# bdaiinstitute/vlfm

Hardware: AMD Instinct MI355X
Metric: env-steps/s (VLM+value-map update), 640x480 RGB-D (higher is better)
Workload: dtype f16 ViT-g (f32 accumulate) + f32 Q-Former (split-f16, 22-bit); f32 confidence + f64 value maps; 1 GPU; configs[1] step x resident envs: BLIP-2 ITC + ValueMap+ObstacleMap+sort_waypoints; envs_per_gpu=256, global_envs=256, map=1000x1000 @ 20 px/m, parallelism=env-sharded x1, tuned_gemms=True, vit_gemm=hip:fc1, attention=hip

## Files before the change

### include/vlfm_amd.h

```cpp
#ifndef VLFM_AMD_H
#define VLFM_AMD_H

#include <stddef.h>
#include <stdint.h>

#ifdef __cplusplus
extern "C" {
#endif

typedef enum {
    VLFM_OK = 0,
    VLFM_ERR_INVALID = -1,
    VLFM_ERR_OUTSIDE_MAP = -2,
    VLFM_ERR_INDEX = -3,
    VLFM_ERR_HIP = -4,
    VLFM_ERR_CAPACITY = -5
} vlfm_status;

enum { VLFM_FUSE_DEFAULT = 0, VLFM_FUSE_REPLACE = 1, VLFM_FUSE_EQUAL_WEIGHTING = 2 };

const char* vlfm_last_error(void);
int vlfm_abi_version(void);

int vlfm_profile_enable(int on);
// ... 124 lines not shown
                                const int32_t* d_hbounds, const int32_t* d_hk, int hksize,
                                const int32_t* d_vbounds, const int32_t* d_vk, int vksize,
                                const float* h_mean3, const float* h_std3, uint8_t* d_tmp, void* d_out,
                                int out_dtype, int patch_size, void* stream);

int vlfm_itc_head_batched(const float* d_proj, int batch, int n_query, int proj_dim,
                          const float* d_text, float* d_out, void* stream);

#define VLFM_ITC_MAX_PROMPTS 8
int vlfm_itc_head_multi(const float* d_proj, int batch, int n_query, int proj_dim, const float* d_text_table, int n_text,
                        const int32_t* d_text_index, int n_prompts, float* d_out, void* stream);

int vlfm_layernorm_bias_f16(const void* d_x, const float* d_channel_bias, const void* d_gamma, const void* d_beta,
                            void* d_y, int rows, int dim, float eps, void* stream);

int vlfm_vit_attention_f16(const void* d_qkv, void* d_out, int batch, int tokens, int heads, int head_dim, float scale,
                           void* stream);

int vlfm_gemm_f16_nt(const void* d_x, const void* d_w, const void* d_bias, void* d_c, int m, int n, int k, int epilogue,
                     void* stream);

int vlfm_gemm_f16_pair_f32_nt(const void* d_x, const void* d_w_pair, const void* d_bias_f32, void* d_out, int m, int n_out, int k,
                              void* stream);

int vlfm_qformer_cross_attention_f32(const void* d_q, const void* d_kv_blocks, void* d_out, int batch, int tokens, int queries,
                                     int heads, int k_block0, int v_block0, int m_total, float scale, void* stream);

int vlfm_gemm_f16_tile_order(int m, int n, int group_m, int* out, int capacity_pairs);
int vlfm_gemm_f16_work_items(int m, int n, int grid, int* out, int capacity_pairs);

int vlfm_split_f32_to_f16_pair(const float* d_src, void* d_hi, void* d_lo, long long count, int* d_overflow, void* stream);
int vlfm_gemm_f32_nt(const float* d_x, const float* d_w, const float* d_bias, const float* d_residual, float* d_c, int m, int n,
                     int k, int activation, int precision, const void* d_w_hi, const void* d_w_lo, int* d_overflow, void* stream);


int vlfm_layernorm_rows_f32(const float* d_x, const float* d_gamma, const float* d_beta, float* d_out, int batch, int height,
                            int width, int channels, int window, float eps, void* stream);
int vlfm_window_reverse_add_f32(float* d_x, const float* d_windows, int batch, int height, int width, int channels, int window,
                                void* stream);
int vlfm_dwconv3x3_nhwc_f32(const float* d_x, const float* d_w9c, const float* d_bias, float* d_out, int batch, int height, int width,
                            int channels, void* stream);
int vlfm_window_attention_f32(const float* d_qkv, const float* d_bias_t, float* d_out, long long windows, int tokens, int heads,
                              float scale, void* stream);
int vlfm_layernorm_rows_shifted_f32(const float* d_x, const float* d_gamma, const float* d_beta, float* d_out, int batch, int height,
                                    int width, int channels, int window, float eps, int shift, int pad_zero, void* stream);
int vlfm_window_reverse_add_shifted_f32(float* d_x, const float* d_windows, int batch, int height, int width, int channels, int window,
                                        int shift, void* stream);
int vlfm_window_attention_masked_f32(const float* d_qkv, const float* d_bias_t, const float* d_mask_t, int windows_per_image, float* d_out,
                                     long long windows, int tokens, int heads, float scale, void* stream);

int vlfm_maxpool2x2_nhwc_f16(const void* d_x, void* d_out, int batch, int height, int width, int channels, void* stream);
int vlfm_conv_nhwc_tile(int pixels, int cin, int cout, int ksize, int* tile_pixels, int* tile_channels);
int vlfm_conv_nhwc_f16(const void* d_x, const void* d_w, const void* d_bias, void* d_out, const void* d_zero, int batch,
                       int height, int width, int cin, int cout, int ksize, int stride, int x_pix_stride,
                       int out_pix_stride, int act, void* stream);

int vlfm_resize_area_tab_host(int ssize, int dsize, int32_t* h_first, int32_t* h_count, float* h_w, int ktaps_capacity);

int vlfm_resize_area_batched(const uint8_t* d_rgb, int n, int height, int width, int out_h, int out_w,
                             const int32_t* d_xfirst, const int32_t* d_xcount, const float* d_xw, int xktaps,
                             const int32_t* d_yfirst, const int32_t* d_ycount, const float* d_yw, int yktaps,
                             void* d_out, int out_dtype, void* stream);

int vlfm_to_tensor_normalize_batched(const uint8_t* d_rgb, int n, int height, int width, const float* h_mean3,
                                     const float* h_std3, float* d_out, void* stream);

// ... 218 lines not shown
```

### vlfm_amd/_lib.py

```python
from __future__ import annotations

import ctypes
import os
import subprocess
from typing import Optional

_HERE = os.path.dirname(os.path.abspath(__file__))
LIB_PATH = os.path.join(_HERE, "libvlfm_amd.so")
SOURCES = ["value_map.hip", "depth_ingest.hip", "depth_holes.hip", "obstacle_map.hip", "vlm_ops.hip", "vit_attention.hip", "qformer_attention.hip", "detect_ops.hip", "object_cloud.hip", "cloud_query.hip", "gemm_f16.hip", "gemm_f32.hip", "conv_nhwc.hip", "sam_ops.hip", "map_render.hip", "jpeg_codec.hip", "jpeg_entropy.hip", "jpeg_decode.hip", "world_render.hip", "geodesic.hip", "map_planner.hip", "host.cpp"]

VLFM_OK = 0
VLFM_ERR_INVALID = -1
VLFM_ERR_OUTSIDE_MAP = -2
VLFM_ERR_INDEX = -3
VLFM_ERR_HIP = -4
VLFM_ERR_CAPACITY = -5

FUSION_TYPES = {"default": 0, "replace": 1, "equal_weighting": 2}


class VmPose(ctypes.Structure):
    _fields_ = [("inv_affine", ctypes.c_double * 6), ("row0", ctypes.c_int32), ("col0", ctypes.c_int32),
                ("env", ctypes.c_int32), ("reserved", ctypes.c_int32)]


class IngestParams(ctypes.Structure):
    _fields_ = [("tf", ctypes.c_double * 12), ("depth_scale", ctypes.c_float), ("depth_offset", ctypes.c_float),
                ("depth_max", ctypes.c_float), ("reserved0", ctypes.c_float), ("fx", ctypes.c_double),
                ("fy", ctypes.c_double), ("min_height", ctypes.c_double), ("max_height", ctypes.c_double),
                ("env", ctypes.c_int32), ("scatter", ctypes.c_int32)]


FOG_MAX_POLY = 80


class FogParams(ctypes.Structure):
    _fields_ = [("env", ctypes.c_int32), ("ax", ctypes.c_int32), ("ay", ctypes.c_int32), ("radius", ctypes.c_int32),
                ("n_poly", ctypes.c_int32), ("reserved", ctypes.c_int32), ("rot_c", ctypes.c_double),
                ("rot_s", ctypes.c_double), ("line_len", ctypes.c_double), ("poly", ctypes.c_longlong * (2 * FOG_MAX_POLY))]


class ScatterJournal(ctypes.Structure):
    _fields_ = [("d_cells", ctypes.c_void_p), ("d_count", ctypes.c_void_p), ("capacity", ctypes.c_int32),
# ... 48 lines not shown
        obj = os.path.join(objdir, os.path.basename(src) + ".o")
        if not os.path.exists(obj) or os.path.getmtime(obj) < max(os.path.getmtime(src), hdr_time):
            cmd = ["hipcc"] + flags + ["-c", src, "-o", obj]
            if verbose:
                print(" ".join(cmd), flush=True)
            subprocess.check_call(cmd)
        return obj

    with ThreadPoolExecutor(max_workers=min(8, len(srcs))) as pool:
        objs = list(pool.map(compile_one, srcs))
    if os.path.exists(LIB_PATH) and all(os.path.getmtime(LIB_PATH) >= os.path.getmtime(o) for o in objs):
        return LIB_PATH
    cmd = ["hipcc", "--offload-arch=gfx950", "-shared", "-fPIC", "-o", LIB_PATH] + objs
    if verbose:
        print(" ".join(cmd), flush=True)
    subprocess.check_call(cmd)
    return LIB_PATH


_lib: Optional[ctypes.CDLL] = None


def lib() -> ctypes.CDLL:
    global _lib
    if _lib is None:
        if not os.path.exists(LIB_PATH):
            raise ImportError(
                f"{LIB_PATH} is missing: build it with `python -c 'import __graft_entry__ as g; g.build()'` "
                "(hipcc --offload-arch=gfx950).  vlfm_amd has no CPU fallback.")
        L = ctypes.CDLL(LIB_PATH)
        vp, ci, cd = ctypes.c_void_p, ctypes.c_int, ctypes.c_double
        L.vlfm_last_error.restype = ctypes.c_char_p
        L.vlfm_abi_version.restype = ci
        L.vlfm_profile_enable.argtypes = [ci]
        L.vlfm_host_wait_mode.argtypes = [ci]
        L.vlfm_profile_read.argtypes = [ctypes.c_char_p, ctypes.POINTER(cd), ctypes.POINTER(ci)]
        L.vlfm_value_map_pose_params.argtypes = [vp, vp, vp, ci, ci, ci, ci, vp, ctypes.POINTER(ci)]
        L.vlfm_cone_template_host.argtypes = [cd, cd, ci, cd, vp, ci, vp, ci, ctypes.POINTER(ci)]
        L.vlfm_tan_table_host.argtypes = [cd, ci, vp]
        L.vlfm_disc_rows_host.argtypes = [ci, vp]
        L.vlfm_cone_template_build.argtypes = [vp, vp, ci, ci, vp, vp, vp]
        L.vlfm_depth_ingest_batched.argtypes = [vp, ci, ci, ci, vp, vp, vp, ci, ci, vp, vp, vp, vp, vp]
        L.vlfm_selftest_div_exact.argtypes = [vp, ci, cd, vp, vp]
        L.vlfm_hole_scratch_bytes.argtypes = [ci, ci, ci, ci, ci]
        L.vlfm_hole_scratch_bytes.restype = ctypes.c_size_t
        L.vlfm_fill_small_holes_batched.argtypes = [vp, vp, ci, ci, ci, cd, vp, ctypes.c_size_t, ci, ci, vp, vp, vp, vp,
                                                    ci, vp, vp]
        L.vlfm_depth_scatter_holes_batched.argtypes = [vp, ci, ci, ci, vp, vp, vp, vp, ci, ci, vp, vp, vp]
        L.vlfm_fill_small_holes_rig_batched.argtypes = [vp, vp, ci, ci, ci, cd, vp, ctypes.c_size_t, ci, ci, vp, vp, vp, vp,
                                                        ci, vp, vp, ci, vp]
        L.vlfm_depth_scatter_holes_rig_batched.argtypes = [vp, ci, ci, ci, vp, vp, vp, vp, ci, ci, vp, vp, vp, vp]
        L.vlfm_layernorm_bias_f16.argtypes = [vp, vp, vp, vp, vp, ci, ci, ctypes.c_float, vp]
        L.vlfm_vit_attention_f16.argtypes = [vp, vp, ci, ci, ci, ci, ctypes.c_float, vp]
        L.vlfm_gemm_f16_nt.argtypes = [vp, vp, vp, vp, ci, ci, ci, ci, vp]
        L.vlfm_gemm_f16_pair_f32_nt.argtypes = [vp, vp, vp, vp, ci, ci, ci, vp]
        L.vlfm_qformer_cross_attention_f32.argtypes = [vp, vp, vp, ci, ci, ci, ci, ci, ci, ci, ctypes.c_float, vp]
        L.vlfm_gemm_f32_nt.argtypes = [vp, vp, vp, vp, vp, ci, ci, ci, ci, ci, vp, vp, vp, vp]
        L.vlfm_split_f32_to_f16_pair.argtypes = [vp, vp, vp, ctypes.c_longlong, vp, vp]
        L.vlfm_layernorm_rows_f32.argtypes = [vp, vp, vp, vp, ci, ci, ci, ci, ci, ctypes.c_float, vp]
        L.vlfm_window_reverse_add_f32.argtypes = [vp, vp, ci, ci, ci, ci, ci, vp]
        L.vlfm_dwconv3x3_nhwc_f32.argtypes = [vp, vp, vp, vp, ci, ci, ci, ci, vp]
        L.vlfm_window_attention_f32.argtypes = [vp, vp, vp, ctypes.c_longlong, ci, ci, ctypes.c_float, vp]
        L.vlfm_layernorm_rows_shifted_f32.argtypes = [vp, vp, vp, vp, ci, ci, ci, ci, ci, ctypes.c_float, ci, ci, vp]
        L.vlfm_window_reverse_add_shifted_f32.argtypes = [vp, vp, ci, ci, ci, ci, ci, ci, vp]
        L.vlfm_window_attention_masked_f32.argtypes = [vp, vp, vp, ci, vp, ctypes.c_longlong, ci, ci, ctypes.c_float, vp]
        L.vlfm_maxpool2x2_nhwc_f16.argtypes = [vp, vp, ci, ci, ci, ci, vp]
        L.vlfm_conv_nhwc_tile.argtypes = [ci, ci, ci, ci, ctypes.POINTER(ci), ctypes.POINTER(ci)]
        L.vlfm_conv_nhwc_f16.argtypes = [vp, vp, vp, vp, vp, ci, ci, ci, ci, ci, ci, ci, ci, ci, ci, vp]
        L.vlfm_value_map_update_fused_batched.argtypes = [vp, ci, vp, vp, vp, ci, vp, vp, ci, vp, vp, ci, ci, ci, cd, cd,
                                                          ci, ci, vp, vp, vp, vp, vp]
        L.vlfm_value_map_update_rig_batched.argtypes = [vp, ci, vp, vp, vp, ci, ci, ci, vp, vp, vp, ci, ci, ci, ci, ci, vp, vp,
                                                        vp, vp]
        L.vlfm_value_map_sort_waypoints_batched.argtypes = [vp, ci, ci, vp, ci, ci, vp, ci, vp, vp]
        L.vlfm_resample_coeffs_host.argtypes = [ci, ci, vp, vp, ci, ctypes.POINTER(ci)]
        L.vlfm_resample_coeffs_filter_host.argtypes = [ci, ci, ci, vp, vp, ci, ctypes.POINTER(ci)]
        L.vlfm_preprocess_sam_batched.argtypes = [vp, ci, ci, ci, ci, ci, vp, vp, ci, vp, vp, ci, vp, vp, ci, vp, vp, vp]
        L.vlfm_preprocess_rgb_batched.argtypes = [vp, ci, ci, ci, ci, vp, vp, ci, vp, vp, ci, vp, vp, vp, vp, ci, ci, vp]
        L.vlfm_itc_head_batched.argtypes = [vp, ci, ci, ci, vp, vp, vp]
        L.vlfm_itc_head_multi.argtypes = [vp, ci, ci, ci, vp, ci, vp, ci, vp, vp]
        cf = ctypes.c_float
        L.vlfm_resize_area_tab_host.argtypes = [ci, ci, vp, vp, vp, ci]
        L.vlfm_resize_area_batched.argtypes = [vp, ci, ci, ci, ci, ci, vp, vp, vp, ci, vp, vp, vp, ci, vp, ci, vp]
        L.vlfm_to_tensor_normalize_batched.argtypes = [vp, ci, ci, ci, vp, vp, vp, vp]
        L.vlfm_nms_scratch_bytes.argtypes = [ci]
        L.vlfm_nms_scratch_bytes.restype = ctypes.c_size_t
        L.vlfm_nms.argtypes = [vp, vp, ci, cf, vp, ctypes.c_size_t, vp, vp, ci, vp]
        L.vlfm_ms_deform_attn.argtypes = [vp, vp, vp, vp, vp, ci, ci, ci, ci, ci, ci, ci, vp, vp]
        L.vlfm_ms_deform_attn_fused.argtypes = [vp, vp, vp, vp, vp, ci, ci, ci, ci, ci, ci, ci, ci, vp, vp]
        L.vlfm_object_cloud_batch_scratch_bytes.argtypes = [ci, ci, ci]
        L.vlfm_object_cloud_batch_scratch_bytes.restype = ctypes.c_size_t
# ... 110 lines not shown
```

### vlfm_amd/csrc/gemm_f32.hip

```cpp
#include <hip/hip_runtime.h>
#include <stdint.h>
#include <stdlib.h>

#include "../../include/vlfm_amd.h"
#include "gelu_f16.h"
#include "mfma.h"
#include "profile.h"
#include "status.h"

namespace vlfm {
namespace g32 {

constexpr int TB = 128;
constexpr int TK = 32;
constexpr int ROWB = TK * 4;
constexpr int OPER = TB * ROWB;
constexpr int BUF = 2 * OPER;
constexpr int EPI_ROW = 272;
constexpr int EPI_WAVE = 64 * EPI_ROW;
constexpr int LDS_EXACT = 4 * EPI_WAVE > 2 * BUF ? 4 * EPI_WAVE : 2 * BUF;

enum { ACT_NONE = 0, ACT_RELU = 1, ACT_GELU = 2 };

struct Args {
    const float* x;
    const float* w;
    const float* bias;
    const float* residual;
    float* c;
    int M, N, K;
    int tiles_m, tiles_n;
    int* overflow;
    const _Float16* w_hi;
    const _Float16* w_lo;
};

__device__ inline void tile_of_block(const Args& a, int& tm, int& tn) {
    const int bid = xcd_contiguous(blockIdx.x, a.tiles_m * a.tiles_n);
    tm = bid / a.tiles_n;
    tn = bid - tm * a.tiles_n;
}

__device__ inline void stage_tile(const Args& a, lds_ptr lds, int buf, int n0, int m0, int k0, int wave, int lane) {
    const int sub = lane >> 3, p = lane & 7;
#pragma unroll
    for (int j = 0; j < 4; j++) {
        const int chunk = wave * 4 + j;
        const int r = chunk * 8 + sub;
        const int s4 = swz128(r, p) >> 2;
        const int rn = min(n0 + r, a.N - 1), rm = min(m0 + r, a.M - 1);
        const float* gw = a.w + (size_t)rn * a.K + k0 + s4;
        const float* gx = a.x + (size_t)rm * a.K + k0 + s4;
        const int dst = __builtin_amdgcn_readfirstlane(buf + chunk * 1024);
        __builtin_amdgcn_global_load_lds((gbl_ptr)gw, lds + dst, 16, 0, 0);
        __builtin_amdgcn_global_load_lds((gbl_ptr)gx, lds + dst + OPER, 16, 0, 0);
    }
}

template <bool SPLIT>
__device__ inline void store_tile(const Args& a, unsigned char* smem, const floatx16 (&acc)[2][2], const floatx16 (&cross)[2][2],
                                  int act, int wave, int wn, int wm, int lane, int m0, int n0) {
    unsigned char* stg = smem + wave * EPI_WAVE;
    const int c32 = lane & 31, h4 = (lane >> 5) * 4;
    floatx4 bias4[2][4];
#pragma unroll
    for (int i = 0; i < 2; i++)
#pragma unroll
        for (int g = 0; g < 4; g++) {
            floatx4 b = {0.f, 0.f, 0.f, 0.f};
            if (a.bias) {
                const int n = n0 + wn * 64 + i * 32 + g * 8 + h4;
                if (n + 4 <= a.N && ((uintptr_t)a.bias & 15) == 0) b = *reinterpret_cast<const floatx4*>(a.bias + n);
                else
                    for (int e = 0; e < 4; e++) b[e] = n + e < a.N ? a.bias[n + e] : 0.f;
            }
            bias4[i][g] = b;
        }
#pragma unroll
    for (int i = 0; i < 2; i++)
#pragma unroll
        for (int g = 0; g < 4; g++) {
            const int nl = i * 32 + g * 8 + h4;
            const floatx4 b = bias4[i][g];
#pragma unroll
            for (int j = 0; j < 2; j++) {
                floatx4 v;
#pragma unroll
                for (int e = 0; e < 4; e++) {
                    float t = acc[i][j][g * 4 + e];
                    if (SPLIT) t = fmaf(cross[i][j][g * 4 + e], 0x1p-11f, t);
                    t += b[e];
                    if (act == ACT_RELU) t = fmaxf(t, 0.f);
                    else if (act == ACT_GELU) t = gelu_erf(t);
                    v[e] = t;
                }
                *reinterpret_cast<floatx4*>(stg + (j * 32 + c32) * EPI_ROW + nl * 4) = v;
            }
        }
    wait_lgkmcnt0();
    const int rsub = lane >> 4, chunk = lane & 15;
    const bool vec = (a.N & 3) == 0;
    const int n = n0 + wn * 64 + chunk * 4;
    const bool fast = vec && n + 4 <= a.N;
    floatx4 r[16], v[16];
#pragma unroll
    for (int it = 0; it < 16; it++) {
        const int m = m0 + wm * 64 + it * 4 + rsub;
        r[it] = floatx4{0.f, 0.f, 0.f, 0.f};
        if (a.residual && fast && m < a.M) r[it] = *reinterpret_cast<const floatx4*>(a.residual + (size_t)m * a.N + n);
    }
#pragma unroll
    for (int it = 0; it < 16; it++) v[it] = *reinterpret_cast<const floatx4*>(stg + (it * 4 + rsub) * EPI_ROW + chunk * 16);
#pragma unroll
    for (int it = 0; it < 16; it++) {
        const int m = m0 + wm * 64 + it * 4 + rsub;
        if (m >= a.M || n >= a.N) continue;
        const size_t at = (size_t)m * a.N + n;
        if (fast) {
            *reinterpret_cast<floatx4*>(a.c + at) = v[it] + r[it];
        } else {
            for (int e = 0; e < 4 && n + e < a.N; e++) a.c[at + e] = v[it][e] + (a.residual ? a.residual[at + e] : 0.f);
        }
    }
}

__global__ __launch_bounds__(256, 2) void gemm_f32_exact_kernel(Args a, int act) {
    extern __shared__ __attribute__((aligned(16))) unsigned char smem[];
    lds_ptr lds = (lds_ptr)smem;
    const int tid = threadIdx.x, lane = tid & 63;
    const int wave = __builtin_amdgcn_readfirstlane(tid >> 6);
    const int wn = wave >> 1, wm = wave & 1;
    int tm, tn;
    tile_of_block(a, tm, tn);
    const int m0 = tm * TB, n0 = tn * TB;
    const int NT = a.K / TK;

    floatx16 acc[2][2];
#pragma unroll
    for (int i = 0; i < 2; i++)
#pragma unroll
        for (int j = 0; j < 2; j++)
#pragma unroll
            for (int e = 0; e < 16; e++) acc[i][j][e] = 0.f;

    stage_tile(a, lds, 0, n0, m0, 0, wave, lane);
    wait_vmcnt<0>();
    __builtin_amdgcn_s_barrier();
    asm volatile("" ::: "memory");
// ... 3 lines not shown
        const int cur = (t & 1) * BUF;
        if (t + 1 < NT) stage_tile(a, lds, cur ^ BUF, n0, m0, (t + 1) * TK, wave, lane);
#pragma unroll
        for (int kk = 0; kk < 4; kk++) {
            const int s = kk * 2 + h;
            floatx4 fa[2], fb[2];
#pragma unroll
            for (int i = 0; i < 2; i++) {
                const int R = wn * 64 + i * 32 + r32;
                fa[i] = *reinterpret_cast<const floatx4*>(smem + cur + R * ROWB + swz128(R, s));
            }
#pragma unroll
            for (int j = 0; j < 2; j++) {
                const int R = wm * 64 + j * 32 + r32;
                fb[j] = *reinterpret_cast<const floatx4*>(smem + cur + OPER + R * ROWB + swz128(R, s));
            }
#pragma unroll
            for (int q = 0; q < 4; q++)
#pragma unroll
                for (int i = 0; i < 2; i++)
#pragma unroll
                    for (int j = 0; j < 2; j++)
                        acc[i][j] = __builtin_amdgcn_mfma_f32_32x32x2f32(fa[i][q], fb[j][q], acc[i][j], 0, 0, 0);
        }
        wait_vmcnt<0>();
        __builtin_amdgcn_s_barrier();
        asm volatile("" ::: "memory");
    }
    store_tile<false>(a, smem, acc, acc, act, wave, wn, wm, lane, m0, n0);
}

constexpr int SROWB = TK * 2;
constexpr int SOPER = TB * SROWB;
constexpr int SBUF = 4 * SOPER;

__device__ inline int sslot(int row, int slot) { return (slot ^ ((row >> 2) & 3)) << 4; }

__device__ inline void split4(const floatx4 v, half4& hi, half4& lo, bool& over) {
#pragma unroll
    for (int e = 0; e < 4; e++) {
        const float a = v[e];
        over |= !(fabsf(a) < 65504.0f);
        const _Float16 hh = (_Float16)a;
        hi[e] = hh;
        lo[e] = (_Float16)((a - (float)hh) * 2048.0f);
    }
}

constexpr int XO = 0, WO = 2 * SOPER;
constexpr int LDS_SPLIT = 4 * EPI_WAVE > 2 * SBUF ? 4 * EPI_WAVE : 2 * SBUF;

__global__ __launch_bounds__(256, 2) void gemm_f32_split_kernel(Args a, int act) {
    extern __shared__ __attribute__((aligned(16))) unsigned char smem[];
    lds_ptr lds = (lds_ptr)smem;
    const int tid = threadIdx.x, lane = tid & 63;
    const int wave = __builtin_amdgcn_readfirstlane(tid >> 6);
    const int wn = wave >> 1, wm = wave & 1;
    int tm, tn;
    tile_of_block(a, tm, tn);
    const int m0 = tm * TB, n0 = tn * TB;
    const int NT = a.K / TK;

    floatx16 acc[2][2], crs[2][2];
#pragma unroll
    for (int i = 0; i < 2; i++)
#pragma unroll
        for (int j = 0; j < 2; j++)
#pragma unroll
            for (int e = 0; e < 16; e++) { acc[i][j][e] = 0.f; crs[i][j][e] = 0.f; }

    floatx4 xr[4];
    bool over = false;
    auto load_x = [&](int k0) {
#pragma unroll
        for (int u = 0; u < 4; u++) {
            const int idx = tid + 256 * u, r = idx >> 3, pc = idx & 7;
            const int rm = min(m0 + r, a.M - 1);
            xr[u] = *reinterpret_cast<const floatx4*>(a.x + (size_t)rm * a.K + k0 + pc * 4);
        }
    };
    auto put_x = [&](int buf) {
#pragma unroll
        for (int u = 0; u < 4; u++) {
            const int idx = tid + 256 * u, r = idx >> 3, pc = idx & 7;
            half4 hi, lo;
            split4(xr[u], hi, lo, over);
            const int off = r * SROWB + sslot(r, pc >> 1) + (pc & 1) * 8;
            *reinterpret_cast<half4*>(smem + buf + XO + off) = hi;
            *reinterpret_cast<half4*>(smem + buf + XO + SOPER + off) = lo;
        }
    };
    auto stage_w = [&](int buf, int k0) {
        const int sub = lane >> 2, p = lane & 3;
#pragma unroll
        for (int j = 0; j < 2; j++) {
            const int chunk = wave * 2 + j;
            const int r = chunk * 16 + sub;
            const int s = p ^ ((r >> 2) & 3);
            const int rn = min(n0 + r, a.N - 1);
            const size_t g = (size_t)rn * a.K + k0 + s * 8;
            const int dst = __builtin_amdgcn_readfirstlane(buf + WO + chunk * 1024);
            __builtin_amdgcn_global_load_lds((gbl_ptr)(a.w_hi + g), lds + dst, 16, 0, 0);
            __builtin_amdgcn_global_load_lds((gbl_ptr)(a.w_lo + g), lds + dst + SOPER, 16, 0, 0);
        }
    };

    load_x(0);
    stage_w(0, 0);
    put_x(0);
    wait_vmcnt<0>();
    wait_lgkmcnt0();
    __builtin_amdgcn_s_barrier();
    asm volatile("" ::: "memory");

    const int r32 = lane & 31, h = lane >> 5;
    for (int t = 0; t < NT; t++) {
        const int cur = (t & 1) * SBUF;
        if (t + 1 < NT) {
            load_x((t + 1) * TK);
            stage_w(cur ^ SBUF, (t + 1) * TK);
        }
#pragma unroll
        for (int kk = 0; kk < 2; kk++) {
            const int s = kk * 2 + h;
            half8 whi[2], wlo[2], xhi[2], xlo[2];
#pragma unroll
            for (int i = 0; i < 2; i++) {
                const int R = wn * 64 + i * 32 + r32, o = cur + WO + R * SROWB + sslot(R, s);
                whi[i] = *reinterpret_cast<const half8*>(smem + o);
                wlo[i] = *reinterpret_cast<const half8*>(smem + o + SOPER);
            }
#pragma unroll
            for (int j = 0; j < 2; j++) {
                const int R = wm * 64 + j * 32 + r32, o = cur + XO + R * SROWB + sslot(R, s);
                xhi[j] = *reinterpret_cast<const half8*>(smem + o);
                xlo[j] = *reinterpret_cast<const half8*>(smem + o + SOPER);
            }
#pragma unroll
            for (int i = 0; i < 2; i++)
#pragma unroll
                for (int j = 0; j < 2; j++) {
                    acc[i][j] = __builtin_amdgcn_mfma_f32_32x32x16_f16(whi[i], xhi[j], acc[i][j], 0, 0, 0);
                    crs[i][j] = __builtin_amdgcn_mfma_f32_32x32x16_f16(whi[i], xlo[j], crs[i][j], 0, 0, 0);
                    crs[i][j] = __builtin_amdgcn_mfma_f32_32x32x16_f16(wlo[i], xhi[j], crs[i][j], 0, 0, 0);
                }
        }
        if (t + 1 < NT) put_x(cur ^ SBUF);
        wait_vmcnt<0>();
        wait_lgkmcnt0();
        __builtin_amdgcn_s_barrier();
        asm volatile("" ::: "memory");
    }
    if (over && a.overflow) atomicOr(a.overflow, 1);
    store_tile<true>(a, smem, acc, crs, act, wave, wn, wm, lane, m0, n0);
}

__global__ void split_f32_kernel(const float* __restrict__ src, _Float16* __restrict__ hi, _Float16* __restrict__ lo, long long n,
                                 int* overflow) {
    const long long i = (long long)blockIdx.x * blockDim.x + threadIdx.x;
    if (i >= n) return;
    const float a = src[i];
    if (!(fabsf(a) < 65504.0f) && overflow) atomicOr(overflow, 1);
    const _Float16 hh = (_Float16)a;
    hi[i] = hh;
    lo[i] = (_Float16)((a - (float)hh) * 2048.0f);
}

}
}

using namespace vlfm;
using namespace vlfm::g32;

extern "C" int vlfm_split_f32_to_f16_pair(const float* d_src, void* d_hi, void* d_lo, long long count, int* d_overflow, void* stream) {
    if (count == 0) return VLFM_OK;
    if (!d_src || !d_hi || !d_lo || count < 0) return fail(VLFM_ERR_INVALID, "split_f32_to_f16_pair: bad argument");
    const long long blocks = (count + 255) / 256;
    VLFM_KLAUNCH(split_f32_kernel, dim3((unsigned)blocks), dim3(256), 0, (hipStream_t)stream, d_src, (_Float16*)d_hi, (_Float16*)d_lo,
                 count, d_overflow);
    return check_launch("split_f32_kernel");
}

extern "C" int vlfm_gemm_f32_nt(const float* d_x, const float* d_w, const float* d_bias, const float* d_residual, float* d_c, int m,
                                int n, int k, int activation, int precision, const void* d_w_hi, const void* d_w_lo,
                                int* d_overflow, void* stream) {
    if (m == 0 || n == 0) return VLFM_OK;
    if (!d_x || !d_w || !d_c || m < 0 || n < 0 || k <= 0 || (k % TK) != 0 || activation < 0 || activation > 2 || precision < 0 ||
        precision > 1)
        return fail(VLFM_ERR_INVALID, "gemm_f32_nt: K must be a multiple of 32, activation 0..2, precision 0..1");
    if (((uintptr_t)d_x | (uintptr_t)d_w | (uintptr_t)d_c | (uintptr_t)d_residual | (uintptr_t)d_w_hi | (uintptr_t)d_w_lo) & 15)
        return fail(VLFM_ERR_INVALID, "gemm_f32_nt: X, W, C, residual and the split weights must be 16-byte aligned");
    if (precision == 1 && (!d_w_hi || !d_w_lo || !d_overflow))
        return fail(VLFM_ERR_INVALID, "gemm_f32_nt: the split form needs the pre-split weights and the overflow flag");
    Args a;
    a.x = d_x; a.w = d_w; a.bias = d_bias; a.residual = d_residual; a.c = d_c;
    a.M = m; a.N = n; a.K = k;
    a.tiles_m = (m + TB - 1) / TB; a.tiles_n = (n + TB - 1) / TB;
    a.overflow = d_overflow; a.w_hi = (const _Float16*)d_w_hi; a.w_lo = (const _Float16*)d_w_lo;
    if ((long long)a.tiles_m * a.tiles_n > 0x7fffffffLL) return fail(VLFM_ERR_CAPACITY, "gemm_f32_nt: too many tiles");
    const dim3 grid(a.tiles_m * a.tiles_n), block(256);
    static LdsOptIn opt_exact, opt_split;
    if (precision == 0) {
        if (LDS_EXACT > 64 * 1024 && !opt_exact.ensure(reinterpret_cast<const void*>(gemm_f32_exact_kernel), LDS_EXACT))
            return fail(VLFM_ERR_HIP, "gemm_f32_nt: cannot opt in to the LDS size");
        VLFM_TIMED("gemm_f32_exact_kernel", stream);
        VLFM_KLAUNCH(gemm_f32_exact_kernel, grid, block, LDS_EXACT, (hipStream_t)stream, a, activation);
        return check_launch("gemm_f32_exact_kernel");
    }
    if (LDS_SPLIT > 64 * 1024 && !opt_split.ensure(reinterpret_cast<const void*>(gemm_f32_split_kernel), LDS_SPLIT))
        return fail(VLFM_ERR_HIP, "gemm_f32_nt: cannot opt in to the LDS size");
    VLFM_TIMED("gemm_f32_split_kernel", stream);
    VLFM_KLAUNCH(gemm_f32_split_kernel, grid, block, LDS_SPLIT, (hipStream_t)stream, a, activation);
    return check_launch("gemm_f32_split_kernel");
}
```

### vlfm_amd/csrc/host.cpp

```cpp
#include <cmath>
#include <cstdint>
#include <cstring>
#include <mutex>
#include <string>

#include "../../include/vlfm_amd.h"
#include "status.h"

namespace vlfm {
static thread_local std::string g_last_error;
void set_last_error(const char* msg) { g_last_error = msg ? msg : ""; }
}

extern "C" const char* vlfm_last_error(void) { return vlfm::g_last_error.c_str(); }
extern "C" int vlfm_abi_version(void) { return 22; }

namespace {

const double kPi = 3.141592653589793238462643383279502884;

inline long round_half_even(double v) { return std::lrint(v); }

float sin_deg_table(int deg) {
    static float tab[451];
    static std::once_flag once;
    std::call_once(once, [] {
        for (int i = 0; i <= 450; i++) tab[i] = (float)(std::round(std::sin(i * kPi / 180.0) * 1e7) / 1e7);
    });
    return tab[deg];
}

}

extern "C" int vlfm_value_map_pose_params(const double* h_tf, const double* h_yaw, const int32_t* h_env, int n,
                                          int map_size, int pixels_per_meter, int template_size,
                                          vlfm_vm_pose* h_out, int* bad_index) {
    if (!h_tf || !h_out || n < 0 || map_size <= 0 || template_size <= 0)
        return vlfm::fail(VLFM_ERR_INVALID, "value_map_pose_params: bad argument");
    const double ppm = (double)pixels_per_meter;
    const int half = template_size / 2;
    for (int k = 0; k < n; k++) {
        const double* tf = h_tf + 16 * k;
        const double yaw = h_yaw ? h_yaw[k] : std::atan2(tf[4], tf[0]);
        const double degrees = (-yaw) * (180.0 / kPi);
        const double ang = degrees * (kPi / 180);
        const double alpha = std::cos(ang), beta = std::sin(ang);
        const double cx = (double)(float)half, cy = (double)(float)half;
        double M[6] = {alpha, beta, (1 - alpha) * cx - beta * cy, -beta, alpha, beta * cx + (1 - alpha) * cy};
// ... 245 lines not shown
```

### vlfm_amd/vlm/ops.py

```python
from __future__ import annotations

import ctypes
from typing import Dict, Optional, Tuple

import numpy as np
import torch

from .. import _lib

CLIP_MEAN = (0.48145466, 0.4578275, 0.40821073)
CLIP_STD = (0.26862954, 0.26130258, 0.27577711)
_DTYPE_CODE = {torch.float32: 0, torch.float16: 1, torch.bfloat16: 2}
_coeff_cache: Dict[Tuple[str, int, int], Tuple[torch.Tensor, torch.Tensor, int]] = {}


def _stream() -> int:
    return torch._C._cuda_getCurrentRawStream(torch._C._cuda_getDevice())


def resample_coeffs(in_size: int, out_size: int, bilinear: bool = False) -> Tuple[np.ndarray, np.ndarray, int]:
    bounds = np.zeros((out_size, 2), np.int32)
    cap = out_size * (2 * int(np.ceil(2.0 * max(1.0, in_size / out_size))) + 1)
    kk = np.zeros(cap, np.int32)
    ks = ctypes.c_int(0)
# ... 341 lines not shown
    if len(_split_cache) > 2048:
        for k in [k for k, v in _split_cache.items() if v[0]() is None]:
            del _split_cache[k]
    w = weight.detach().contiguous()
    hi = torch.empty(w.shape, dtype=torch.float16, device=w.device)
    lo = torch.empty_like(hi)
    bad = torch.zeros(1, dtype=torch.int32, device=w.device)
    _lib.check(_lib.lib().vlfm_split_f32_to_f16_pair(w.data_ptr(), hi.data_ptr(), lo.data_ptr(), w.numel(), bad.data_ptr(),
                                                     _stream()), "split_f32")
    gemm_f32_overflow_flag(w.device, owner).bitwise_or_(bad)
    _split_cache[key] = [weakref.ref(weight), tensor_version(weight), weight.data_ptr(), hi, lo, bad, False, owner]
    return hi, lo


def split_weights_bad(device, owner: str = "") -> bool:
    d = torch.device(device)
    entries = [v for v in _split_cache.values() if v[7] == owner and v[0]() is not None and v[5].device.type == d.type
               and (d.index is None or v[5].device.index == d.index)]
    if not entries:
        return False
    verdict = torch.cat([v[5] for v in entries]).cpu().tolist()
    for v, b in zip(entries, verdict):
        v[6] = bool(b)
    return any(verdict)


def linear_f32_supported(x: torch.Tensor, weight: torch.Tensor) -> bool:
    k = weight.shape[1]
    return (x.is_cuda and x.dtype == torch.float32 and weight.dtype == torch.float32 and k % 32 == 0 and x.shape[-1] == k
            and weight.shape[0] >= 32 and x.numel() // k >= 64 and not torch.is_grad_enabled())


def linear_f32(x: torch.Tensor, weight: torch.Tensor, bias=None, act=None, residual=None, precision: str = "exact",
               out=None, owner: str = "") -> torch.Tensor:
    K = weight.shape[1]
    N = weight.shape[0]
    lead = x.shape[:-1]
    x2 = x.reshape(-1, K)
    if not x2.is_contiguous() or x2.data_ptr() % 16:
        x2 = x2.contiguous()
    w = weight if weight.is_contiguous() else weight.contiguous()
    M = x2.shape[0]
    if out is None:
        out = torch.empty((M, N), dtype=torch.float32, device=x.device)
    res = None
    if residual is not None:
        res = residual.reshape(M, N)
        if not res.is_contiguous() or res.data_ptr() % 16:
            res = res.contiguous()
    b = None
    if bias is not None:
        b = bias if bias.is_contiguous() else bias.contiguous()
    prec = GEMM_F32_PRECISION[precision]
    hi = lo = None
    if prec == 1:
        hi, lo = split_weight(w, owner)
    _lib.check(_lib.lib().vlfm_gemm_f32_nt(x2.data_ptr(), w.data_ptr(), b.data_ptr() if b is not None else None,
                                           res.data_ptr() if res is not None else None, out.data_ptr(), M, N, K, _ACT32[act], prec,
                                           hi.data_ptr() if hi is not None else None, lo.data_ptr() if lo is not None else None,
                                           gemm_f32_overflow_flag(x.device, owner).data_ptr(), _stream()), "gemm_f32_nt")
    return out.view(*lead, N)


_tuned_gemms_state = None


def use_tuned_gemms() -> bool:
    global _tuned_gemms_state
    if _tuned_gemms_state is None:
        import os

        path = os.path.join(os.path.dirname(os.path.dirname(os.path.abspath(__file__))), "tunableop_results.csv")
        ok = False
        if os.environ.get("VLFM_TUNED_GEMMS", "1") != "0" and os.path.exists(path) and torch.cuda.is_available():
            try:
                import torch.cuda.tunable as tunable

                import tempfile

                tunable.enable(True)
                tunable.tuning_enable(False)
                tunable.set_filename(os.path.join(tempfile.gettempdir(), f"vlfm_amd_tunableop_{os.getpid()}.csv"))
                ok = bool(tunable.read_file(path))
            except Exception as exc:
                import warnings

                warnings.warn(f"tuned GEMM solutions not loaded ({type(exc).__name__}: {exc})")
                ok = False
        _tuned_gemms_state = ok
    return _tuned_gemms_state
```

Measured before the change: 1688 env-steps/s.

## Add 96-wide N tile to split-f16 f32 GEMM chosen by wave quantization

Templates the split-precision f32 GEMM kernel on its N tile width and adds a 96-column variant using a 3x1 wave layout, plus explicit MFMA/LDS-read scheduling barriers for it. A host heuristic picks 96 or 128 from how many waves of tiles fill twice the CU count, aiming to reduce tail-wave underutilization in the Q-Former GEMMs. The W staging is restructured per plane. It also adds an ABI version check on library load. The 96 tile has lower arithmetic intensity per block and may lose where quantization is not the bottleneck.

After: 1686 env-steps/s. No clear change (-0.1%).

```diff
diff --git a/include/vlfm_amd.h b/include/vlfm_amd.h
--- a/include/vlfm_amd.h
+++ b/include/vlfm_amd.h
@@ -180,6 +180,10 @@
 int vlfm_split_f32_to_f16_pair(const float* d_src, void* d_hi, void* d_lo, long long count, int* d_overflow, void* stream);
 int vlfm_gemm_f32_nt(const float* d_x, const float* d_w, const float* d_bias, const float* d_residual, float* d_c, int m, int n,
                      int k, int activation, int precision, const void* d_w_hi, const void* d_w_lo, int* d_overflow, void* stream);
+int vlfm_gemm_f32_split_tile_n(int m, int n, int cus);
+int vlfm_gemm_f32_nt_tile(const float* d_x, const float* d_w, const float* d_bias, const float* d_residual, float* d_c, int m, int n,
+                          int k, int activation, int precision, const void* d_w_hi, const void* d_w_lo, int* d_overflow, int tile_n,
+                          void* stream);
 
 
 int vlfm_layernorm_rows_f32(const float* d_x, const float* d_gamma, const float* d_beta, float* d_out, int batch, int height,
diff --git a/vlfm_amd/_lib.py b/vlfm_amd/_lib.py
--- a/vlfm_amd/_lib.py
+++ b/vlfm_amd/_lib.py
@@ -9,6 +9,7 @@
 LIB_PATH = os.path.join(_HERE, "libvlfm_amd.so")
 SOURCES = ["value_map.hip", "depth_ingest.hip", "depth_holes.hip", "obstacle_map.hip", "vlm_ops.hip", "vit_attention.hip", "qformer_attention.hip", "detect_ops.hip", "object_cloud.hip", "cloud_query.hip", "gemm_f16.hip", "gemm_f32.hip", "conv_nhwc.hip", "sam_ops.hip", "map_render.hip", "jpeg_codec.hip", "jpeg_entropy.hip", "jpeg_decode.hip", "world_render.hip", "geodesic.hip", "map_planner.hip", "host.cpp"]
 
+ABI_VERSION = 23
 VLFM_OK = 0
 VLFM_ERR_INVALID = -1
 VLFM_ERR_OUTSIDE_MAP = -2
@@ -123,6 +124,9 @@
         vp, ci, cd = ctypes.c_void_p, ctypes.c_int, ctypes.c_double
         L.vlfm_last_error.restype = ctypes.c_char_p
         L.vlfm_abi_version.restype = ci
+        if L.vlfm_abi_version() != ABI_VERSION:
+            raise ImportError(f"{LIB_PATH} has ABI {L.vlfm_abi_version()}, this package binds ABI {ABI_VERSION}: rebuild it with "
+                              "`python -c 'import __graft_entry__ as g; g.build()'`")
         L.vlfm_profile_enable.argtypes = [ci]
         L.vlfm_host_wait_mode.argtypes = [ci]
         L.vlfm_profile_read.argtypes = [ctypes.c_char_p, ctypes.POINTER(cd), ctypes.POINTER(ci)]
@@ -147,6 +151,8 @@
         L.vlfm_gemm_f16_pair_f32_nt.argtypes = [vp, vp, vp, vp, ci, ci, ci, vp]
         L.vlfm_qformer_cross_attention_f32.argtypes = [vp, vp, vp, ci, ci, ci, ci, ci, ci, ci, ctypes.c_float, vp]
         L.vlfm_gemm_f32_nt.argtypes = [vp, vp, vp, vp, vp, ci, ci, ci, ci, ci, vp, vp, vp, vp]
+        L.vlfm_gemm_f32_nt_tile.argtypes = [vp, vp, vp, vp, vp, ci, ci, ci, ci, ci, vp, vp, vp, ci, vp]
+        L.vlfm_gemm_f32_split_tile_n.argtypes = [ci, ci, ci]
         L.vlfm_split_f32_to_f16_pair.argtypes = [vp, vp, vp, ctypes.c_longlong, vp, vp]
         L.vlfm_layernorm_rows_f32.argtypes = [vp, vp, vp, vp, ci, ci, ci, ci, ci, ctypes.c_float, vp]
         L.vlfm_window_reverse_add_f32.argtypes = [vp, vp, ci, ci, ci, ci, ci, vp]
diff --git a/vlfm_amd/csrc/gemm_f32.hip b/vlfm_amd/csrc/gemm_f32.hip
--- a/vlfm_amd/csrc/gemm_f32.hip
+++ b/vlfm_amd/csrc/gemm_f32.hip
@@ -16,9 +16,9 @@
 constexpr int ROWB = TK * 4;
 constexpr int OPER = TB * ROWB;
 constexpr int BUF = 2 * OPER;
-constexpr int EPI_ROW = 272;
-constexpr int EPI_WAVE = 64 * EPI_ROW;
-constexpr int LDS_EXACT = 4 * EPI_WAVE > 2 * BUF ? 4 * EPI_WAVE : 2 * BUF;
+constexpr int epi_row(int ni) { return ni * 128 + 16; }
+constexpr int epi_wave(int ni, int nj) { return nj * 32 * epi_row(ni); }
+constexpr int LDS_EXACT = 4 * epi_wave(2, 2) > 2 * BUF ? 4 * epi_wave(2, 2) : 2 * BUF;
 
 enum { ACT_NONE = 0, ACT_RELU = 1, ACT_GELU = 2 };
 
@@ -57,19 +57,20 @@
     }
 }
 
-template <bool SPLIT>
-__device__ inline void store_tile(const Args& a, unsigned char* smem, const floatx16 (&acc)[2][2], const floatx16 (&cross)[2][2],
+template <bool SPLIT, int NI, int NJ>
+__device__ inline void store_tile(const Args& a, unsigned char* smem, const floatx16 (&acc)[NI][NJ], const floatx16 (&cross)[NI][NJ],
                                   int act, int wave, int wn, int wm, int lane, int m0, int n0) {
-    unsigned char* stg = smem + wave * EPI_WAVE;
+    constexpr int EPI_ROW = epi_row(NI), WN = NI * 32, WM = NJ * 32;
+    unsigned char* stg = smem + wave * epi_wave(NI, NJ);
     const int c32 = lane & 31, h4 = (lane >> 5) * 4;
-    floatx4 bias4[2][4];
-#pragma unroll
-    for (int i = 0; i < 2; i++)
+    floatx4 bias4[NI][4];
+#pragma unroll
+    for (int i = 0; i < NI; i++)
 #pragma unroll
         for (int g = 0; g < 4; g++) {
             floatx4 b = {0.f, 0.f, 0.f, 0.f};
             if (a.bias) {
-                const int n = n0 + wn * 64 + i * 32 + g * 8 + h4;
+                const int n = n0 + wn * WN + i * 32 + g * 8 + h4;
                 if (n + 4 <= a.N && ((uintptr_t)a.bias & 15) == 0) b = *reinterpret_cast<const floatx4*>(a.bias + n);
                 else
                     for (int e = 0; e < 4; e++) b[e] = n + e < a.N ? a.bias[n + e] : 0.f;
@@ -77,13 +78,13 @@
             bias4[i][g] = b;
         }
 #pragma unroll
-    for (int i = 0; i < 2; i++)
+    for (int i = 0; i < NI; i++)
 #pragma unroll
         for (int g = 0; g < 4; g++) {
             const int nl = i * 32 + g * 8 + h4;
             const floatx4 b = bias4[i][g];
 #pragma unroll
-            for (int j = 0; j < 2; j++) {
+            for (int j = 0; j < NJ; j++) {
                 floatx4 v;
 #pragma unroll
                 for (int e = 0; e < 4; e++) {
@@ -98,22 +99,27 @@
             }
         }
     wait_lgkmcnt0();
-    const int rsub = lane >> 4, chunk = lane & 15;
+    constexpr int LPR = NI * 8, ITERS = WM * LPR / 64;
     const bool vec = (a.N & 3) == 0;
-    const int n = n0 + wn * 64 + chunk * 4;
-    const bool fast = vec && n + 4 <= a.N;
-    floatx4 r[16], v[16];
-#pragma unroll
-    for (int it = 0; it < 16; it++) {
-        const int m = m0 + wm * 64 + it * 4 + rsub;
+    floatx4 r[ITERS], v[ITERS];
+#pragma unroll
+    for (int it = 0; it < ITERS; it++) {
+        const int row = (it * 64 + lane) / LPR, chunk = (it * 64 + lane) % LPR;
+        const int m = m0 + wm * WM + row, n = n0 + wn * WN + chunk * 4;
+        const bool fast = vec && n + 4 <= a.N;
         r[it] = floatx4{0.f, 0.f, 0.f, 0.f};
         if (a.residual && fast && m < a.M) r[it] = *reinterpret_cast<const floatx4*>(a.residual + (size_t)m * a.N + n);
     }
 #pragma unroll
-    for (int it = 0; it < 16; it++) v[it] = *reinterpret_cast<const floatx4*>(stg + (it * 4 + rsub) * EPI_ROW + chunk * 16);
-#pragma unroll
-    for (int it = 0; it < 16; it++) {
-        const int m = m0 + wm * 64 + it * 4 + rsub;
+    for (int it = 0; it < ITERS; it++) {
+        const int row = (it * 64 + lane) / LPR, chunk = (it * 64 + lane) % LPR;
+        v[it] = *reinterpret_cast<const floatx4*>(stg + row * EPI_ROW + chunk * 16);
+    }
+#pragma unroll
+    for (int it = 0; it < ITERS; it++) {
+        const int row = (it * 64 + lane) / LPR, chunk = (it * 64 + lane) % LPR;
+        const int m = m0 + wm * WM + row, n = n0 + wn * WN + chunk * 4;
+        const bool fast = vec && n + 4 <= a.N;
         if (m >= a.M || n >= a.N) continue;
         const size_t at = (size_t)m * a.N + n;
         if (fast) {
@@ -183,7 +189,6 @@
 
 constexpr int SROWB = TK * 2;
 constexpr int SOPER = TB * SROWB;
-constexpr int SBUF = 4 * SOPER;
 
 __device__ inline int sslot(int row, int slot) { return (slot ^ ((row >> 2) & 3)) << 4; }
 
@@ -198,25 +203,38 @@
     }
 }
 
-constexpr int XO = 0, WO = 2 * SOPER;
-constexpr int LDS_SPLIT = 4 * EPI_WAVE > 2 * SBUF ? 4 * EPI_WAVE : 2 * SBUF;
-
+template <int TN>
+struct SplitTile {
+    static constexpr int NI = TN == 128 ? 2 : 3, NJ = TN == 128 ? 2 : 1;
+    static constexpr int WAVES_M = TB / (32 * NJ);
+    static constexpr int WOPER = TN * SROWB;
+    static constexpr int XO = 0, WO = 2 * SOPER;
+    static constexpr int BUF = 2 * SOPER + 2 * WOPER;
+    static constexpr int EPI = 4 * epi_wave(NI, NJ);
+    static constexpr int LDS = EPI > 2 * BUF ? EPI : 2 * BUF;
+    static_assert(TN == 128 || TN == 96, "tile widths of the split form");
+    static_assert(4 / WAVES_M * NI * 32 == TN && (TN / 16 * 2) % 4 == 0, "wavefront layout and W staging cover the tile");
+};
+
+template <int TN>
 __global__ __launch_bounds__(256, 2) void gemm_f32_split_kernel(Args a, int act) {
+    using G = SplitTile<TN>;
+    constexpr int NI = G::NI, NJ = G::NJ, XO = G::XO, WO = G::WO, WOPER = G::WOPER, SBUF = G::BUF;
     extern __shared__ __attribute__((aligned(16))) unsigned char smem[];
     lds_ptr lds = (lds_ptr)smem;
     const int tid = threadIdx.x, lane = tid & 63;
     const int wave = __builtin_amdgcn_readfirstlane(tid >> 6);
-    const int wn = wave >> 1, wm = wave & 1;
+    const int wn = wave / G::WAVES_M, wm = wave % G::WAVES_M;
     int tm, tn;
     tile_of_block(a, tm, tn);
-    const int m0 = tm * TB, n0 = tn * TB;
+    const int m0 = tm * TB, n0 = tn * TN;
     const int NT = a.K / TK;
 
-    floatx16 acc[2][2], crs[2][2];
-#pragma unroll
-    for (int i = 0; i < 2; i++)
-#pragma unroll
-        for (int j = 0; j < 2; j++)
+    floatx16 acc[NI][NJ], crs[NI][NJ];
+#pragma unroll
+    for (int i = 0; i < NI; i++)
+#pragma unroll
+        for (int j = 0; j < NJ; j++)
 #pragma unroll
             for (int e = 0; e < 16; e++) { acc[i][j][e] = 0.f; crs[i][j][e] = 0.f; }
 
@@ -242,17 +260,18 @@
         }
     };
     auto stage_w = [&](int buf, int k0) {
+        constexpr int PER = TN / 16 * 2 / 4;
         const int sub = lane >> 2, p = lane & 3;
 #pragma unroll
-        for (int j = 0; j < 2; j++) {
-            const int chunk = wave * 2 + j;
+        for (int j = 0; j < PER; j++) {
+            const int item = wave * PER + j;
+            const int chunk = item >> 1, plane = item & 1;
             const int r = chunk * 16 + sub;
             const int s = p ^ ((r >> 2) & 3);
             const int rn = min(n0 + r, a.N - 1);
             const size_t g = (size_t)rn * a.K + k0 + s * 8;
-            const int dst = __builtin_amdgcn_readfirstlane(buf + WO + chunk * 1024);
-            __builtin_amdgcn_global_load_lds((gbl_ptr)(a.w_hi + g), lds + dst, 16, 0, 0);
-            __builtin_amdgcn_global_load_lds((gbl_ptr)(a.w_lo + g), lds + dst + SOPER, 16, 0, 0);
+            const int dst = __builtin_amdgcn_readfirstlane(buf + WO + plane * WOPER + chunk * 1024);
+            __builtin_amdgcn_global_load_lds((gbl_ptr)((plane ? a.w_lo : a.w_hi) + g), lds + dst, 16, 0, 0);
         }
     };
 
@@ -274,27 +293,36 @@
 #pragma unroll
         for (int kk = 0; kk < 2; kk++) {
             const int s = kk * 2 + h;
-            half8 whi[2], wlo[2], xhi[2], xlo[2];
-#pragma unroll
-            for (int i = 0; i < 2; i++) {
-                const int R = wn * 64 + i * 32 + r32, o = cur + WO + R * SROWB + sslot(R, s);
+            half8 whi[NI], wlo[NI], xhi[NJ], xlo[NJ];
+#pragma unroll
+            for (int i = 0; i < NI; i++) {
+                const int R = wn * (NI * 32) + i * 32 + r32, o = cur + WO + R * SROWB + sslot(R, s);
                 whi[i] = *reinterpret_cast<const half8*>(smem + o);
-                wlo[i] = *reinterpret_cast<const half8*>(smem + o + SOPER);
-            }
-#pragma unroll
-            for (int j = 0; j < 2; j++) {
-                const int R = wm * 64 + j * 32 + r32, o = cur + XO + R * SROWB + sslot(R, s);
+                wlo[i] = *reinterpret_cast<const half8*>(smem + o + WOPER);
+            }
+#pragma unroll
+            for (int j = 0; j < NJ; j++) {
+                const int R = wm * (NJ * 32) + j * 32 + r32, o = cur + XO + R * SROWB + sslot(R, s);
                 xhi[j] = *reinterpret_cast<const half8*>(smem + o);
                 xlo[j] = *reinterpret_cast<const half8*>(smem + o + SOPER);
             }
 #pragma unroll
-            for (int i = 0; i < 2; i++)
-#pragma unroll
-                for (int j = 0; j < 2; j++) {
+            for (int i = 0; i < NI; i++)
+#pragma unroll
+                for (int j = 0; j < NJ; j++) {
                     acc[i][j] = __builtin_amdgcn_mfma_f32_32x32x16_f16(whi[i], xhi[j], acc[i][j], 0, 0, 0);
                     crs[i][j] = __builtin_amdgcn_mfma_f32_32x32x16_f16(whi[i], xlo[j], crs[i][j], 0, 0, 0);
                     crs[i][j] = __builtin_amdgcn_mfma_f32_32x32x16_f16(wlo[i], xhi[j], crs[i][j], 0, 0, 0);
                 }
+        }
+        if constexpr (TN == 96) {
+            __builtin_amdgcn_sched_group_barrier(0x100, 8, 0);
+#pragma unroll
+            for (int u = 0; u < 8; u++) {
+                __builtin_amdgcn_sched_group_barrier(0x008, 1, 0);
+                __builtin_amdgcn_sched_group_barrier(0x100, 1, 0);
+            }
+            __builtin_amdgcn_sched_group_barrier(0x008, 10, 0);
         }
         if (t + 1 < NT) put_x(cur ^ SBUF);
         wait_vmcnt<0>();
@@ -332,13 +360,36 @@
     return check_launch("split_f32_kernel");
 }
 
-extern "C" int vlfm_gemm_f32_nt(const float* d_x, const float* d_w, const float* d_bias, const float* d_residual, float* d_c, int m,
-                                int n, int k, int activation, int precision, const void* d_w_hi, const void* d_w_lo,
-                                int* d_overflow, void* stream) {
+extern "C" int vlfm_gemm_f32_split_tile_n(int m, int n, int cus) {
+    if (m <= 0 || n <= 0 || cus <= 0) return 128;
+    const long long slots = 2LL * cus, tiles_m = (m + TB - 1) / TB;
+    const long long t128 = tiles_m * ((n + 127) / 128), t96 = tiles_m * ((n + 95) / 96);
+    if (t96 < slots) return 128;
+    return (t96 + slots - 1) / slots <= (t128 + slots - 1) / slots ? 96 : 128;
+}
+
+template <int TN>
+static int launch_split(Args a, int activation, hipStream_t stream) {
+    using G = SplitTile<TN>;
+    a.tiles_n = (a.N + TN - 1) / TN;
+    if ((long long)a.tiles_m * a.tiles_n > 0x7fffffffLL) return fail(VLFM_ERR_CAPACITY, "gemm_f32_nt: too many tiles");
+    static LdsOptIn opt;
+    if (G::LDS > 64 * 1024 && !opt.ensure(reinterpret_cast<const void*>(gemm_f32_split_kernel<TN>), G::LDS))
+        return fail(VLFM_ERR_HIP, "gemm_f32_nt: cannot opt in to the LDS size");
+    VLFM_TIMED("gemm_f32_split_kernel", stream);
+    VLFM_KLAUNCH(gemm_f32_split_kernel<TN>, dim3(a.tiles_m * a.tiles_n), dim3(256), G::LDS, stream, a, activation);
+    return check_launch("gemm_f32_split_kernel");
+}
+
+extern "C" int vlfm_gemm_f32_nt_tile(const float* d_x, const float* d_w, const float* d_bias, const float* d_residual, float* d_c, int m,
+                                     int n, int k, int activation, int precision, const void* d_w_hi, const void* d_w_lo,
+                                     int* d_overflow, int tile_n, void* stream) {
     if (m == 0 || n == 0) return VLFM_OK;
     if (!d_x || !d_w || !d_c || m < 0 || n < 0 || k <= 0 || (k % TK) != 0 || activation < 0 || activation > 2 || precision < 0 ||
         precision > 1)
         return fail(VLFM_ERR_INVALID, "gemm_f32_nt: K must be a multiple of 32, activation 0..2, precision 0..1");
+    if (tile_n != 0 && tile_n != 128 && !(tile_n == 96 && precision == 1))
+        return fail(VLFM_ERR_INVALID, "gemm_f32_nt: tile_n is 0 (chosen here), 128, or 96 for the split form");
     if (((uintptr_t)d_x | (uintptr_t)d_w | (uintptr_t)d_c | (uintptr_t)d_residual | (uintptr_t)d_w_hi | (uintptr_t)d_w_lo) & 15)
         return fail(VLFM_ERR_INVALID, "gemm_f32_nt: X, W, C, residual and the split weights must be 16-byte aligned");
     if (precision == 1 && (!d_w_hi || !d_w_lo || !d_overflow))
@@ -348,19 +399,23 @@
     a.M = m; a.N = n; a.K = k;
     a.tiles_m = (m + TB - 1) / TB; a.tiles_n = (n + TB - 1) / TB;
     a.overflow = d_overflow; a.w_hi = (const _Float16*)d_w_hi; a.w_lo = (const _Float16*)d_w_lo;
-    if ((long long)a.tiles_m * a.tiles_n > 0x7fffffffLL) return fail(VLFM_ERR_CAPACITY, "gemm_f32_nt: too many tiles");
-    const dim3 grid(a.tiles_m * a.tiles_n), block(256);
-    static LdsOptIn opt_exact, opt_split;
     if (precision == 0) {
+        if ((long long)a.tiles_m * a.tiles_n > 0x7fffffffLL) return fail(VLFM_ERR_CAPACITY, "gemm_f32_nt: too many tiles");
+        const dim3 grid(a.tiles_m * a.tiles_n), block(256);
+        static LdsOptIn opt_exact;
         if (LDS_EXACT > 64 * 1024 && !opt_exact.ensure(reinterpret_cast<const void*>(gemm_f32_exact_kernel), LDS_EXACT))
             return fail(VLFM_ERR_HIP, "gemm_f32_nt: cannot opt in to the LDS size");
         VLFM_TIMED("gemm_f32_exact_kernel", stream);
         VLFM_KLAUNCH(gemm_f32_exact_kernel, grid, block, LDS_EXACT, (hipStream_t)stream, a, activation);
         return check_launch("gemm_f32_exact_kernel");
     }
-    if (LDS_SPLIT > 64 * 1024 && !opt_split.ensure(reinterpret_cast<const void*>(gemm_f32_split_kernel), LDS_SPLIT))
-        return fail(VLFM_ERR_HIP, "gemm_f32_nt: cannot opt in to the LDS size");
-    VLFM_TIMED("gemm_f32_split_kernel", stream);
-    VLFM_KLAUNCH(gemm_f32_split_kernel, grid, block, LDS_SPLIT, (hipStream_t)stream, a, activation);
-    return check_launch("gemm_f32_split_kernel");
-}
+    if (tile_n == 0) tile_n = vlfm_gemm_f32_split_tile_n(m, n, device_cu_count());
+    return tile_n == 96 ? launch_split<96>(a, activation, (hipStream_t)stream) : launch_split<128>(a, activation, (hipStream_t)stream);
+}
+
+extern "C" int vlfm_gemm_f32_nt(const float* d_x, const float* d_w, const float* d_bias, const float* d_residual, float* d_c, int m,
+                                int n, int k, int activation, int precision, const void* d_w_hi, const void* d_w_lo,
+                                int* d_overflow, void* stream) {
+    return vlfm_gemm_f32_nt_tile(d_x, d_w, d_bias, d_residual, d_c, m, n, k, activation, precision, d_w_hi, d_w_lo, d_overflow, 0,
+                                 stream);
+}
diff --git a/vlfm_amd/csrc/host.cpp b/vlfm_amd/csrc/host.cpp
--- a/vlfm_amd/csrc/host.cpp
+++ b/vlfm_amd/csrc/host.cpp
@@ -13,7 +13,7 @@
 }
 
 extern "C" const char* vlfm_last_error(void) { return vlfm::g_last_error.c_str(); }
-extern "C" int vlfm_abi_version(void) { return 22; }
+extern "C" int vlfm_abi_version(void) { return 23; }
 
 namespace {
 
diff --git a/vlfm_amd/vlm/ops.py b/vlfm_amd/vlm/ops.py
--- a/vlfm_amd/vlm/ops.py
+++ b/vlfm_amd/vlm/ops.py
@@ -397,7 +397,7 @@
 
 
 def linear_f32(x: torch.Tensor, weight: torch.Tensor, bias=None, act=None, residual=None, precision: str = "exact",
-               out=None, owner: str = "") -> torch.Tensor:
+               out=None, owner: str = "", _tile_n: int = 0) -> torch.Tensor:
     K = weight.shape[1]
     N = weight.shape[0]
     lead = x.shape[:-1]
@@ -420,10 +420,11 @@
     hi = lo = None
     if prec == 1:
         hi, lo = split_weight(w, owner)
-    _lib.check(_lib.lib().vlfm_gemm_f32_nt(x2.data_ptr(), w.data_ptr(), b.data_ptr() if b is not None else None,
-                                           res.data_ptr() if res is not None else None, out.data_ptr(), M, N, K, _ACT32[act], prec,
-                                           hi.data_ptr() if hi is not None else None, lo.data_ptr() if lo is not None else None,
-                                           gemm_f32_overflow_flag(x.device, owner).data_ptr(), _stream()), "gemm_f32_nt")
+    _lib.check(_lib.lib().vlfm_gemm_f32_nt_tile(x2.data_ptr(), w.data_ptr(), b.data_ptr() if b is not None else None,
+                                                res.data_ptr() if res is not None else None, out.data_ptr(), M, N, K, _ACT32[act], prec,
+                                                hi.data_ptr() if hi is not None else None, lo.data_ptr() if lo is not None else None,
+                                                gemm_f32_overflow_flag(x.device, owner).data_ptr(), _tile_n, _stream()),
+               "gemm_f32_nt")
     return out.view(*lead, N)
 
 
```
